# RuanJohn/Mava

Measured on AMD Instinct MI355X. Metric: env-steps/sec (whole node), ff_mappo RWARE tiny-4ag, higher is better.
Workload: dtype f32 via 2 x f16 split operands on the MFMA (3 products, f32 accumulate); 1 GPU; ff_mappo RWARE tiny-4ag-shaped synthetic obs, 4096 envs/GPU (update_batch_size=1 x num_envs=4096), rollout_length=128, ppo_epochs=4, num_minibatches=2, agents=4, obs=70/264, actions=5, one step = one PPO update = 524288 env-steps per GPU; parallelism=dp1

## Files before the change

mava_amd/csrc/ppo_train_h2.hip:

```cpp
#include "h2_core.h"
#include "ppo_train_task.h"
#include "ctx.h"

#include <type_traits>

#ifndef MAVA_GW_DEPTH
#define MAVA_GW_DEPTH 0
#endif
#define GW_DEPTH MAVA_GW_DEPTH
#ifndef MAVA_GW_DEPTH_WIDE
#define MAVA_GW_DEPTH_WIDE 0
#endif

namespace {

using namespace h2;

constexpr int STATS_BLOCKS = 128;

#ifdef MAVA_STAMPS
#define STAMP_DECL unsigned long long st_prev = __builtin_readcyclecounter(), st_acc[16] = {0, 0, 0, 0, 0, 0, 0, 0, 0, 0, 0, 0, 0, 0, 0, 0};
#define STAMP(i)                                                    \
  do {                                                              \
    __builtin_amdgcn_sched_barrier(0);                              \
    const unsigned long long st_now = __builtin_readcyclecounter(); \
    st_acc[i] += st_now - st_prev;                                  \
    st_prev = st_now;                                               \
    __builtin_amdgcn_sched_barrier(0);                              \
  } while (0)
#else
#define STAMP_DECL
#define STAMP(i)
#endif

struct H2Layout {
  int h1, dz2, dz1, w2, xs, xs_plane, xs_row, dy, yp, agg, small, end;
};

template <int NO, int S1, bool WIDE>
H2Layout make_h2_layout(bool actor) {
  constexpr int KT1 = (S1 + 1) / 2;
  H2Layout L;
  L.h1 = 0;
  L.dz2 = L.h1 + IMG_BYTES;
  L.dz1 = L.dz2 + IMG_BYTES;
  L.w2 = L.dz1 + IMG_BYTES;
  L.xs = L.w2 + 4 * IMG_BYTES;
  L.xs_row = 2 * 32 * KT1 + 16;
  L.xs_plane = 32 * L.xs_row;
  L.dy = L.xs + (WIDE ? 1 : 2) * 2 * L.xs_plane;
  L.yp = actor ? L.dz2 : L.dz1;
  L.agg = L.dy + (actor ? 2 * DY_PLANE : 0);
  L.small = L.agg + 8 * 33 * 4;
  L.small = (L.small + 15) & ~15;
  L.end = L.small + (128 + 32 + 16 + 128) * 4;
  return L;
}
constexpr int W2_PLANE = 128 * SW_ROW;
constexpr int W1_RING = 3;

template <int STEPS>
__global__ __launch_bounds__(256) void pack_w1_kernel(const float* __restrict__ P, int din, uint4* __restrict__ out, float scale) {
  pack_w1_body<STEPS>(P, din, out, threadIdx.x, scale);
}

template <int NO, int S1, bool ACTOR, bool WIDE, int XV, int ROLE>
__device__ __forceinline__ void h2_body(const TrainTask& tk, const H2Layout& L, const uint4* __restrict__ w1p, u8* lds) {
  static_assert(!WIDE || S1 % W1_RING == 0, "WIDE: S1 must be a multiple of the W1 ring depth");
  static_assert((ROLE == 0) == !WIDE, "roles 1 / 2 belong to WIDE launches");
  constexpr bool CHAIN = ROLE != 2, LOADER = ROLE != 1;
#if defined(MAVA_NO_W2_RESIDENT) || defined(MAVA_W2_RESIDENT_P4)
  constexpr bool W2_RESIDENT = false;
#else
  constexpr bool W2_RESIDENT = !WIDE && NO <= 16;
#endif
#ifdef MAVA_W2_RESIDENT_P4
  constexpr bool W2_RES4 = !WIDE && ACTOR && NO <= 16;
#else
  constexpr bool W2_RES4 = false;
#endif
  constexpr int NTHR = WIDE ? 512 : 256;
  constexpr float WS = ACTOR ? 1.0f : W_SCALE_CRITIC, WU = 1.0f / WS;
  constexpr int KT1 = (S1 + 1) / 2;
  u8* const H1I = lds + L.h1;
  u8* const DZ2I = lds + L.dz2;
  u8* const DZ1I = lds + L.dz1;
  u8* const H2I = lds + L.dz1;
  u8* const W2I = lds + L.w2;
  u8* const DYI = lds + L.dy;
  float* const YP = reinterpret_cast<float*>(lds + L.yp);
  float* const AGG = reinterpret_cast<float*>(lds + L.agg);
  float* const B2s = reinterpret_cast<float*>(lds + L.small);
  float* const B3s = B2s + 128;
  float* const misc = B3s + 32;
  float* const W3s = misc + 16;
  const int xs_row = L.xs_row, xs_plane = L.xs_plane;

  int tid = threadIdx.x & 255;
  int lane = tid & 63, w = tid >> 6, h = lane >> 5, r = lane & 31;
  int srow = tid >> 3, l8 = tid & 7;
  const int din = tk.din, no = tk.no;
  const long R = (!ACTOR && tk.agg > 1) ? (long)tk.Rb : (long)tk.Rb * tk.A;
  const float invR = 1.0f / (float)((long)tk.Rb * tk.A);
  constexpr int NPC = (32 * KT1 / XV + 7) / 8;
  constexpr int NR = NPC * XV;

  for (int i = threadIdx.x * 16; i < L.end; i += NTHR * 16) *reinterpret_cast<uint4*>(lds + i) = make_uint4(0, 0, 0, 0);
  __syncthreads();
  const float* const P = tk.params;
  const int oW2 = mlp_off_w2(din), oW3 = mlp_off_w3(din);
  if (CHAIN) {
    if (tid < 128) B2s[tid] = P[mlp_off_b2(din) + tid];
    if (tid < no) B3s[tid] = P[mlp_off_b3(din, no) + tid];
    if (!ACTOR && tid < 128) W3s[tid] = P[oW3 + tid];
    if (tid < (WIDE ? 32 : 64)) {
      const int b = tid >> 5, row = tid & 31;
      *reinterpret_cast<_Float16*>(lds + L.xs + b * 2 * xs_plane + row * xs_row + 2 * din) = (_Float16)1.0f;
    }
    {
      const int n = tid & 127, k0 = 64 * (tid >> 7);
      float carry = 0.0f;
#pragma unroll 8
      for (int k = k0; k < k0 + 64; ++k) {
        _Float16 x0, x1;
        split1_carry(P[oW2 + k * MLP_H + n] * WS, carry, x0, x1);
        const int o = sw_off(k, n >> 3) + 2 * (n & 7);
        *reinterpret_cast<_Float16*>(W2I + o) = x0;
        *reinterpret_cast<_Float16*>(W2I + W2_PLANE + o) = x1;
      }
    }
    if (ACTOR && tid == 0) {
      double s1 = 0.0, s2 = 0.0;
      for (int i = 0; i < STATS_BLOCKS; ++i) { s1 += tk.stats[2 * i]; s2 += tk.stats[2 * i + 1]; }
      const double mean = s1 / (double)R;
      double var = s2 / (double)R - mean * mean;
      if (var < 0.0) var = 0.0;
      misc[0] = (float)mean;
      misc[1] = 1.0f / ((float)sqrt(var) + 1e-8f);
    }
  }
  constexpr int S_LO = (WIDE && !CHAIN) ? S1 / 2 : 0, S_HI = (WIDE && CHAIN) ? S1 / 2 : S1, RL = S_HI - S_LO;
  static_assert(!WIDE || ((S1 / 2) % W1_RING == 0 && (S1 - S1 / 2) % W1_RING == 0), "WIDE: both halves must be multiples of the ring");
  constexpr int NW1 = WIDE ? W1_RING : (CHAIN ? S1 : 1);
  Frag W1f[NW1];
  const uint4* w1p_lane = w1p + 2 * (w * 64 + lane);
  typedef unsigned u32x4 __attribute__((ext_vector_type(4)));
  typedef const __attribute__((address_space(1))) u32x4* w1_gptr;
  auto w1_fetch = [&](int s) -> Frag {
    const w1_gptr g = (w1_gptr)w1p_lane;
    Frag f;
    f.hi = __builtin_bit_cast(half8, g[512 * s]);
    f.lo = __builtin_bit_cast(half8, g[512 * s + 1]);
    return f;
  };
  float w1_carry = 0.0f;
#pragma unroll
  for (int s = 0; s < (CHAIN ? NW1 : 0); ++s) {
    if (WIDE) {
      W1f[s] = w1_fetch(S_LO + s);
    } else {
      float v[8];
#pragma unroll
      for (int e = 0; e < 8; ++e) {
        const int k = 16 * s + 8 * h + e;
        v[e] = (k <= din) ? P[k * MLP_H + 32 * w + r] * WS : 0.0f;
      }
      W1f[s] = split8_carry(v, w1_carry);
    }
  }
  Frag W3h[2];
#pragma unroll
  for (int s = 0; s < ((CHAIN && ACTOR) ? 2 : 0); ++s) {
    float v[8];
#pragma unroll
    for (int e = 0; e < 8; ++e) {
      const int f = 32 * w + 16 * s + 8 * (e >> 2) + 4 * h + (e & 3);
      v[e] = (r < no) ? P[oW3 + f * no + r] * W3_SCALE : 0.0f;
    }
    W3h[s] = split8(v);
  }
  constexpr int ND = NO > 16 ? 2 : 1;
  Frag W3d[ND];
  if (CHAIN && ACTOR) {
#pragma unroll
    for (int s = 0; s < ND; ++s) {
      float v[8];
#pragma unroll
      for (int e = 0; e < 8; ++e) {
        const int o = 16 * s + 8 * h + e;
        v[e] = (o < no) ? P[oW3 + (32 * w + r) * no + o] * W3_SCALE : 0.0f;
      }
      W3d[s] = split8(v);
    }
  }
  __syncthreads();
  const float adv_mean = ACTOR ? misc[0] : 0.0f;
  const float adv_rstd = ACTOR ? misc[1] : 0.0f;

  f32x16 gW1[LOADER ? KT1 : 1], gW2[4], gW3;
#pragma unroll
  for (int t = 0; t < (LOADER ? KT1 : 1); ++t)
#pragma unroll
    for (int q = 0; q < 16; ++q) gW1[t][q] = 0.0f;
#pragma unroll
  for (int t = 0; t < 4; ++t)
#pragma unroll
    for (int q = 0; q < 16; ++q) gW2[t][q] = 0.0f;
#pragma unroll
  for (int q = 0; q < 16; ++q) gW3[q] = 0.0f;
  float ab2[16], aW3r[ACTOR ? 1 : 16];
#pragma unroll
  for (int q = 0; q < 16; ++q) ab2[q] = 0.0f;
#pragma unroll
  for (int q = 0; q < (ACTOR ? 1 : 16); ++q) aW3r[q] = 0.0f;
  float ab3 = 0.0f, loss_a = 0.0f, loss_b = 0.0f;

  constexpr int NP = ACTOR ? NO / 8 : 1;
  constexpr int GR = ACTOR ? 64 / NO : 32;
  const int lo = ACTOR ? (lane & (NO - 1)) : 0;
  auto loss_row = [&](int q) -> int { return ACTOR ? (8 * w + q * GR + lane / NO) : r; };
  const int slot = 2 * w + h;
  uint32_t slot_c = (!ACTOR && tk.agg > 1) ? (uint32_t)(slot < tk.agg ? slot : 0) : 0u;
  auto load_row = [&](long fr, int& act, float& f0, float& f1, uint32_t& m) {
    if (ACTOR) {
      act = tk.action[fr];
      f0 = tk.old_logp[fr];
      f1 = tk.adv[fr];
      const uint8_t* mk = (tk.mask != nullptr && lo < no) ? (tk.mask + fr * no + lo) : nullptr;
      m = 1u;
      if (mk != nullptr) m = *mk;
    } else {
      act = 0;
      const long fa = (tk.agg > 1) ? (long)((uint32_t)fr * (uint32_t)tk.agg + slot_c) : fr;
      f0 = tk.old_value[fa];
      f1 = tk.targets[fa];
      m = 0u;
    }
  };
  const uint32_t Au = (!ACTOR && tk.agg > 1) ? 1u : (uint32_t)tk.A;
  const uint32_t q_step = 32u * gridDim.x, b_step = q_step / Au, a_step = q_step % Au;
  const uint32_t b_last = (uint32_t)(R - 1) / Au, a_last = (uint32_t)(R - 1) % Au;
  struct Cursor { uint32_t q, b, a; };
  auto cursor_at = [&](int rr) {
    Cursor c;
    c.q = 32u * blockIdx.x + (uint32_t)rr;
    c.b = c.q / Au;
    c.a = c.q - c.b * Au;
    return c;
  };
  auto cursor_advance = [&](Cursor& c) {
    c.q += q_step; c.b += b_step; c.a += a_step;
    if (c.a >= Au) { c.a -= Au; c.b += 1u; }
  };
  auto cursor_gather = [&](const Cursor& c, int32_t& p_raw, uint32_t& a_out) {
    const bool in = c.q < (uint32_t)R;
    const uint32_t b = in ? c.b : b_last;
    a_out = in ? c.a : a_last;
    p_raw = tk.idx ? tk.idx[b] : (int32_t)(tk.idx_base + (long)b);
  };
  auto stage_row = [&](int32_t p_raw, uint32_t a) -> uint32_t {
    const uint32_t fr = (uint32_t)p_raw * Au + a;
    return (tk.xshare == 1) ? fr : ((uint32_t)tk.xshare == Au ? (uint32_t)p_raw : fr / (uint32_t)tk.xshare);
  };
  const int nv = din / XV;
  auto stage_issue = [&](uint32_t xrow_idx, float (&xr)[NR]) {
    const float* xrow = tk.x + (long)xrow_idx * din;
#pragma unroll
    for (int i = 0; i < NPC; ++i) {
      const int c = l8 + 8 * i;
      const int cc = (c < nv) ? c : 0;
      if (XV == 4) {
        const float4 v = reinterpret_cast<const float4*>(xrow)[cc];
        xr[4 * i] = v.x; xr[4 * i + 1] = v.y; xr[4 * i + 2] = v.z; xr[4 * i + 3] = v.w;
      } else if (XV == 2) {
        const float2 v = reinterpret_cast<const float2*>(xrow)[cc];
        xr[2 * i] = v.x; xr[2 * i + 1] = v.y;
      } else {
        xr[i] = xrow[cc];
      }
    }
  };
  u8* const xs_dummy = reinterpret_cast<u8*>(misc + 8);
  unsigned* const xflag = reinterpret_cast<unsigned*>(misc + 2);
  int tpar = 0;
  auto stage_commit = [&](auto hi_only_tag, auto flag_tag, u8* dst, const float (&xr)[NR], int flag_slot) {
    constexpr bool HI_ONLY = decltype(hi_only_tag)::value, FLAG = decltype(flag_tag)::value;
    u8* base = dst + srow * xs_row;
    uint32_t lo_any = 0;
#pragma unroll
    for (int i = 0; i < NPC; ++i) {
      const int c = l8 + 8 * i;
      const bool ok = c < nv;
      u8* qa = ok ? (base + 2 * XV * c) : xs_dummy;
      u8* qb = ok ? (base + xs_plane + 2 * XV * c) : xs_dummy;
      if (XV == 4) {
        half4 a, b;
#pragma unroll
        for (int e = 0; e < 4; ++e) { _Float16 x0, x1; split1(xr[4 * i + e], x0, x1); a[e] = x0; b[e] = x1; }
        *reinterpret_cast<half4*>(qa) = a;
        if constexpr (!HI_ONLY) *reinterpret_cast<half4*>(qb) = b;
        if constexpr (FLAG) {
          const uint2 bb = __builtin_bit_cast(uint2, b);
          lo_any |= (bb.x | bb.y) & 0x7FFF7FFFu;
        }
      } else if (XV == 2) {
        typedef _Float16 half2v __attribute__((ext_vector_type(2)));
        half2v a, b;
#pragma unroll
        for (int e = 0; e < 2; ++e) { _Float16 x0, x1; split1(xr[2 * i + e], x0, x1); a[e] = x0; b[e] = x1; }
        *reinterpret_cast<half2v*>(qa) = a;
        if constexpr (!HI_ONLY) *reinterpret_cast<half2v*>(qb) = b;
        if constexpr (FLAG) lo_any |= __builtin_bit_cast(uint32_t, b) & 0x7FFF7FFFu;
      } else {
        _Float16 x0, x1;
        split1(xr[i], x0, x1);
        *reinterpret_cast<_Float16*>(qa) = x0;
        if constexpr (!HI_ONLY) *reinterpret_cast<_Float16*>(qb) = x1;
        if constexpr (FLAG) lo_any |= (uint32_t)__builtin_bit_cast(uint16_t, x1) & 0x7FFFu;
      }
    }
    if constexpr (FLAG) {
      if (lo_any != 0) xflag[flag_slot] = 1u;
    }
  };
  using std::false_type;
  using std::true_type;
  constexpr bool VERSIONED = WIDE && !ACTOR;
  using versioned_tag = std::bool_constant<VERSIONED>;

  const long ntiles = (R + 31) / 32;
  long it = blockIdx.x;
  float xr[NR];
  int r_act[NP] = {}, n_act[NP] = {};
  float r_f0[NP] = {}, r_f1[NP] = {}, n_f0[NP] = {}, n_f1[NP] = {};
  uint32_t r_m[NP] = {}, n_m[NP] = {};
  Cursor cs = cursor_at(srow), cl[NP];
#pragma unroll
  for (int q = 0; q < NP; ++q) cl[q] = cursor_at(loss_row(q));
  int32_t ps_next = 0, pl_next[NP] = {};
  uint32_t as_next = 0, al_next[NP] = {};
  if (it < ntiles) {
    if (LOADER) {
      cursor_gather(cs, ps_next, as_next);
      stage_issue(stage_row(ps_next, as_next), xr);
    }
    if (CHAIN) {
#pragma unroll
      for (int q = 0; q < NP; ++q) {
        cursor_gather(cl[q], pl_next[q], al_next[q]);
        load_row((long)((uint32_t)pl_next[q] * Au + al_next[q]), r_act[q], r_f0[q], r_f1[q], r_m[q]);
      }
    }
    if (LOADER) {
      stage_commit(false_type{}, versioned_tag{}, lds + L.xs, xr, 0);
      cursor_advance(cs);
    }
    if (CHAIN) {
#pragma unroll
      for (int q = 0; q < NP; ++q) cursor_advance(cl[q]);
    }
    if (it + gridDim.x < ntiles) {
      if (LOADER) {
        cursor_gather(cs, ps_next, as_next);
        cursor_advance(cs);
      }
      if (CHAIN) {
#pragma unroll
        for (int q = 0; q < NP; ++q) cursor_gather(cl[q], pl_next[q], al_next[q]);
#pragma unroll
        for (int q = 0; q < NP; ++q) cursor_advance(cl[q]);
      }
    }
  }
  __syncthreads();

  SwRow rowB = sw_row(r, h);
  SwTr trS = sw_tr(lane);
  const int i16 = lane & 15, tq = i16 >> 2, tp = i16 & 3, g1 = (lane >> 4) & 1;
  int trX = (8 * h + tq) * xs_row + 2 * (16 * g1 + 4 * tp);
  const int trD = (8 * h + tq) * DY_ROW + 2 * (16 * g1 + 4 * tp);
  SwRow w2row = sw_row(32 * w + r, h);
  int buf = 0;
  Frag w2r[(W2_RESIDENT || W2_RES4) ? 8 : 1];
  if constexpr (W2_RESIDENT) {
#pragma unroll
    for (int s = 0; s < 8; ++s) w2r[s] = sw_read_tr(W2I, W2_PLANE, trS, s, w);
  }
  if constexpr (W2_RES4) {
#pragma unroll
    for (int s = 0; s < 8; ++s) w2r[s] = sw_read_row(W2I, W2_PLANE, w2row, s);
  }

  STAMP_DECL
  bool exact = false;
  unsigned n_exact = 0;
  auto tile_body = [&](auto exact_tag) __attribute__((always_inline)) {
    constexpr bool EXACT = decltype(exact_tag)::value;
    static_assert(!EXACT || VERSIONED, "the exact-input loop belongs to the wide critic");
    STAMP(14);
    const bool valid = (it * 32 + r) < R;
    const long itn = it + gridDim.x;
    const bool have_next = itn < ntiles;
    if constexpr (EXACT && LOADER) {
      if (tid == 0) xflag[tpar ^ 1] = 0u;
    }
    uint32_t xrow_next = LOADER ? stage_row(ps_next, as_next) : 0u;
    uint32_t fr_next[NP];
#pragma unroll
    for (int q = 0; q < NP; ++q) fr_next[q] = CHAIN ? ((uint32_t)pl_next[q] * Au + al_next[q]) : 0u;
    if (LOADER) asm volatile("" : "+v"(xrow_next));
    if (CHAIN) {
#pragma unroll
      for (int q = 0; q < NP; ++q) asm volatile("" : "+v"(fr_next[q]));
    }
    const u8* const XSI = lds + L.xs + (EXACT ? tpar : 2 * buf) * xs_plane;

    f32x16 acc;
    uint32_t relu1 = 0;
    if constexpr (WIDE) asm volatile("" : "+v"(w1p_lane));
    if constexpr (CHAIN || WIDE) {
#pragma unroll
    for (int q = 0; q < 16; ++q) acc[q] = 0.0f;
    if constexpr (WIDE && !CHAIN) {
#pragma unroll
      for (int s = 0; s < NW1; ++s) W1f[s] = w1_fetch(S_LO + s);
    }
    Frag xb;
    xb.hi = *reinterpret_cast<const half8*>(XSI + r * xs_row + 16 * h + 32 * S_LO);
    if constexpr (!EXACT) xb.lo = *reinterpret_cast<const half8*>(XSI + xs_plane + r * xs_row + 16 * h + 32 * S_LO);
#pragma unroll
    for (int j = 0; j < RL; ++j) {
      const Frag b = xb;
      if (j + 1 < RL) {
        xb.hi = *reinterpret_cast<const half8*>(XSI + r * xs_row + 16 * h + 32 * (S_LO + j + 1));
        if constexpr (!EXACT) xb.lo = *reinterpret_cast<const half8*>(XSI + xs_plane + r * xs_row + 16 * h + 32 * (S_LO + j + 1));
      }
      if constexpr (EXACT) {
        acc = __builtin_amdgcn_mfma_f32_32x32x16_f16(W1f[j % NW1].lo, b.hi, acc, 0, 0, 0);
        acc = __builtin_amdgcn_mfma_f32_32x32x16_f16(W1f[j % NW1].hi, b.hi, acc, 0, 0, 0);
      } else {
        acc = mfma3(W1f[j % NW1], b, acc);
      }
      if (WIDE) {
        if (j >= 1 && j - 1 + W1_RING < RL) W1f[(j - 1) % NW1] = w1_fetch(S_LO + j - 1 + W1_RING);
      }
      __builtin_amdgcn_sched_barrier(0);
    }
    }
    if constexpr (WIDE) {
      float4* const xch = reinterpret_cast<float4*>(DZ2I) + (w * 4) * 64 + lane;
      if constexpr (LOADER) {
#pragma unroll
        for (int g = 0; g < 4; ++g) xch[g * 64] = make_float4(acc[4 * g], acc[4 * g + 1], acc[4 * g + 2], acc[4 * g + 3]);
      }
      __syncthreads();
      if constexpr (CHAIN) {
#pragma unroll
        for (int g = 0; g < 4; ++g) {
          const float4 v = xch[g * 64];
          acc[4 * g] += v.x; acc[4 * g + 1] += v.y; acc[4 * g + 2] += v.z; acc[4 * g + 3] += v.w;
        }
      }
    }
    if constexpr (CHAIN) {
    STAMP(0);
#pragma unroll
    for (int q = 0; q < 16; ++q) {
      acc[q] = fmaxf(ACTOR ? acc[q] : acc[q] * WU, 0.0f);
      relu1 |= (acc[q] > 0.0f) ? (1u << q) : 0u;
    }
    {
      half4 ph[4], pl[4];
      sw_write_image(H1I, r, w, h, acc, ph, pl);
    }
    }
    STAMP(1);
    if constexpr (WIDE && LOADER) {
      stage_issue(have_next ? xrow_next : 0u, xr);
    }
    if constexpr (WIDE && CHAIN) {
#pragma unroll
      for (int q = 0; q < NP; ++q) {
        asm volatile("" : "+v"(fr_next[q]));
        asm volatile("" : "+v"(cl[q].q), "+v"(cl[q].b), "+v"(cl[q].a));
      }
      asm volatile("" : "+v"(slot_c));
    }
    if constexpr (WIDE && CHAIN) {
      if (have_next) {
        const bool more = itn + gridDim.x < ntiles;
        Cursor c_old[NP];
        if (more) {
#pragma unroll
          for (int q = 0; q < NP; ++q) { c_old[q] = cl[q]; cursor_advance(cl[q]); }
        }
        __builtin_amdgcn_sched_barrier(0);
#pragma unroll
        for (int q = 0; q < NP; ++q) load_row((long)fr_next[q], n_act[q], n_f0[q], n_f1[q], n_m[q]);
        __builtin_amdgcn_sched_barrier(0);
        if (more) {
#pragma unroll
          for (int q = 0; q < NP; ++q) cursor_gather(c_old[q], pl_next[q], al_next[q]);
        }
      }
    } else if (have_next) {
      if (LOADER && !WIDE) stage_issue(xrow_next, xr);
      const bool more = itn + gridDim.x < ntiles;
      if (more) {
        if (LOADER) {
          cursor_gather(cs, ps_next, as_next);
          cursor_advance(cs);
        }
        if (CHAIN) {
          Cursor c_old[NP];
#pragma unroll
          for (int q = 0; q < NP; ++q) { c_old[q] = cl[q]; cursor_advance(cl[q]); }
          __builtin_amdgcn_sched_barrier(0);
#pragma unroll
          for (int q = 0; q < NP; ++q) cursor_gather(c_old[q], pl_next[q], al_next[q]);
        }
      }
      if (CHAIN) {
#pragma unroll
        for (int q = 0; q < NP; ++q) load_row((long)fr_next[q], n_act[q], n_f0[q], n_f1[q], n_m[q]);
      }
    }
    if constexpr (WIDE && CHAIN) {
      __builtin_amdgcn_sched_barrier(0);
#pragma unroll
      for (int s2 = 0; s2 < NW1; ++s2) W1f[s2] = w1_fetch(S_LO + s2);
      __builtin_amdgcn_sched_barrier(0);
    }
    STAMP(2);
    __syncthreads();
    STAMP(3);

    f32x16 h2;
    uint32_t relu2 = 0;
    if constexpr (CHAIN) {
#pragma unroll
    for (int q = 0; q < 16; ++q) h2[q] = B2s[32 * w + (q & 3) + 8 * (q >> 2) + 4 * h] * WS;
    {
      Frag an;
      if constexpr (!W2_RESIDENT) an = sw_read_tr(W2I, W2_PLANE, trS, 0, w);
      Frag bn = sw_read_row(H1I, SW_PLANE, rowB, 0);
#pragma unroll
      for (int s = 0; s < 8; ++s) {
        const Frag a = W2_RESIDENT ? w2r[s] : an, b = bn;
        if (s + 1 < 8) {
          if constexpr (!W2_RESIDENT) an = sw_read_tr(W2I, W2_PLANE, trS, s + 1, w);
          bn = sw_read_row(H1I, SW_PLANE, rowB, s + 1);
        }
        h2 = mfma3(a, b, h2);
        __builtin_amdgcn_sched_barrier(0);
      }
    }
    STAMP(4);
#pragma unroll
    for (int q = 0; q < 16; ++q) {
      h2[q] = fmaxf(ACTOR ? h2[q] : h2[q] * WU, 0.0f);
      relu2 |= (h2[q] > 0.0f) ? (1u << q) : 0u;
    }
    if (!ACTOR) {
      float4 w3g[4];
#pragma unroll
      for (int g = 0; g < 4; ++g) w3g[g] = *reinterpret_cast<const float4*>(W3s + 32 * w + 4 * h + 8 * g);
      float part = 0.0f;
#pragma unroll
      for (int q = 0; q < 16; ++q) {
        const float4 t = w3g[q >> 2];
        const float w3 = (q & 3) == 0 ? t.x : (q & 3) == 1 ? t.y : (q & 3) == 2 ? t.z : t.w;
        part = fmaf(h2[q], w3, part);
      }
      part += __shfl_xor(part, 32, 64);
      if (h == 0) YP[(w * 32 + r) * (NO + 1)] = part;
    } else {
      half4 ph[4], pl[4];
      sw_write_image(H2I, r, w, h, h2, ph, pl);
      f32x16 yacc;
#pragma unroll
      for (int q = 0; q < 16; ++q) yacc[q] = 0.0f;
#pragma unroll
      for (int s = 0; s < 2; ++s) {
        Frag b;
        b.hi = __builtin_shufflevector(ph[2 * s], ph[2 * s + 1], 0, 1, 2, 3, 4, 5, 6, 7);
        b.lo = __builtin_shufflevector(pl[2 * s], pl[2 * s + 1], 0, 1, 2, 3, 4, 5, 6, 7);
        yacc = mfma3(W3h[s], b, yacc);
      }
#pragma unroll
      for (int q = 0; q < 16; ++q) {
        const int o = (q & 3) + 8 * (q >> 2) + 4 * h;
        if ((q & 3) + 8 * (q >> 2) < NO) {
          if (o < NO) YP[(w * 32 + r) * (NO + 1) + o] = yacc[q] * W3_UNSCALE;
        }
      }
    }
    }
    STAMP(5);
    __syncthreads();
    STAMP(6);
    if constexpr (EXACT && LOADER) {
      stage_commit(true_type{}, true_type{}, lds + L.xs + (tpar ^ 1) * xs_plane, xr, tpar ^ 1);
    }

    f32x16 dz;
    float dy0 = 0.0f;
    if constexpr (CHAIN) {
    if (ACTOR) {
      const float lo_c = 1.0f - tk.clip_eps, hi_c = 1.0f + tk.clip_eps;
#pragma unroll
      for (int q = 0; q < NP; ++q) {
        const int row = loss_row(q);
        const bool rvalid = (it * 32 + row) < R;
        const float* yp = YP + row * (NO + 1) + lo;
        const float y = (((yp[0] + yp[32 * (NO + 1)]) + yp[2 * 32 * (NO + 1)]) + yp[3 * 32 * (NO + 1)]) + B3s[lo];
        const bool legal = (lo < no) && (r_m[q] != 0u);
        const float z = legal ? y : -FLT_MAX;
        auto fmax_op = [](float a, float b) { return fmaxf(a, b); };
        auto add_op = [](float a, float b) { return a + b; };
        const float mx = group_allreduce<NO>(z, fmax_op);
        const float se = group_allreduce<NO>(expf(z - mx), add_op);
        const float logp = (mx == -FLT_MAX) ? ((lo < no) ? -logf((float)no) : -FLT_MAX) : z - (mx + logf(se));
        const float pr = expf(logp);
        const float ent = group_allreduce<NO>((pr > 0.0f) ? -(pr * logp) : 0.0f, add_op);
        const int act = r_act[q];
        const float lp = group_allreduce<NO>((lo == act) ? logp : 0.0f, add_op);
        const float gae = (r_f1[q] - adv_mean) * adv_rstd;
        const float ratio = expf(lp - r_f0[q]);
        const float rc = fminf(fmaxf(ratio, lo_c), hi_c);
        const float l1 = ratio * gae, l2 = rc * gae;
        const float pg = -fminf(l1, l2);
        const bool inside = (ratio >= lo_c) && (ratio <= hi_c);
        const float g1 = (l1 < l2) ? 1.0f : ((l1 == l2) ? 0.5f : 0.0f);
        const float g2 = inside ? (1.0f - g1) : 0.0f;
        const float dlp = rvalid ? (-(g1 + g2) * gae * ratio) : 0.0f;
        const float ec = rvalid ? tk.ent_coef : 0.0f;
        const float oh = (lo == act) ? 1.0f : 0.0f;
        const float pl2 = (pr > 0.0f) ? logp : 0.0f;
        float dyo = dlp * (oh - pr) + ec * pr * (pl2 + ent);
        if (z == -FLT_MAX) dyo = 0.0f;
        _Float16 da, db;
        split1(dyo, da, db);
        *reinterpret_cast<_Float16*>(DYI + row * DY_ROW + 2 * lo) = da;
        *reinterpret_cast<_Float16*>(DYI + DY_PLANE + row * DY_ROW + 2 * lo) = db;
        ab3 += dyo;
        if (rvalid && lo == 0) {
          loss_a += pg * invR;
          loss_b += ent * invR;
        }
      }
    } else {
      const float* yp = YP + r * (NO + 1);
      const float v = (((yp[0] + yp[32 * (NO + 1)]) + yp[2 * 32 * (NO + 1)]) + yp[3 * 32 * (NO + 1)]) + B3s[0];
      const float ov = r_f0[0], tg = r_f1[0];
      const float diff = v - ov;
      const float vclip = ov + fminf(fmaxf(diff, -tk.clip_eps), tk.clip_eps);
      const float e1 = v - tg, e2 = vclip - tg;
      const float l1 = e1 * e1, l2 = e2 * e2;
      const bool inside = (diff >= -tk.clip_eps) && (diff <= tk.clip_eps);
      const float g1 = (l1 > l2) ? 1.0f : ((l1 == l2) ? 0.5f : 0.0f);
      const float g2 = inside ? (1.0f - g1) : 0.0f;
      dy0 = valid ? (tk.vf_coef * (g1 * e1 + g2 * e2)) : 0.0f;
      if (tk.agg > 1) {
        const bool mine = valid && slot < tk.agg;
        dy0 = mine ? dy0 : 0.0f;
        if (mine) {
          loss_a += 0.5f * fmaxf(l1, l2) * invR;
          ab3 += dy0;
        }
        AGG[slot * 33 + r] = dy0;
      } else if (valid && w == 0 && h == 0) {
        loss_a += 0.5f * fmaxf(l1, l2) * invR;
        ab3 += dy0;
      }
    }
    }
    STAMP(7);
    __syncthreads();
    STAMP(15);
    if constexpr (CHAIN) {
    if (ACTOR) {
#pragma unroll
      for (int s = 0; s < 2; ++s) {
        const Frag a = read_tr_frag(DYI + trD + 16 * s * DY_ROW, DY_PLANE, DY_ROW);
        const Frag b = sw_read_tr(H2I, SW_PLANE, trS, s, w);
        gW3 = mfma3(a, b, gW3);
      }
#pragma unroll
      for (int q = 0; q < 16; ++q) dz[q] = 0.0f;
#pragma unroll
      for (int s = 0; s < ND; ++s) {
        const Frag b = read_row_frag(DYI, DY_PLANE, r * DY_ROW + 32 * s + 16 * h);
        dz = mfma3(W3d[s], b, dz);
      }
#pragma unroll
      for (int q = 0; q < 16; ++q) {
        dz[q] = ((relu2 >> q) & 1u) ? dz[q] * W3_UNSCALE : 0.0f;
        ab2[q] += dz[q];
      }
    } else {
      float4 w3g[4];
#pragma unroll
      for (int g = 0; g < 4; ++g) w3g[g] = *reinterpret_cast<const float4*>(W3s + 32 * w + 4 * h + 8 * g);
      if (tk.agg > 1) {
        float av[8];
#pragma unroll
        for (int a = 0; a < 8; ++a) av[a] = AGG[a * 33 + r];
        float sum = 0.0f;
#pragma unroll
        for (int a = 0; a < 8; ++a) sum += av[a];
        dy0 = sum;
      }
#pragma unroll
      for (int q = 0; q < 16; ++q) {
        const float4 t = w3g[q >> 2];
        const float w3 = (q & 3) == 0 ? t.x : (q & 3) == 1 ? t.y : (q & 3) == 2 ? t.z : t.w;
        const float v = w3 * dy0;
        dz[q] = ((relu2 >> q) & 1u) ? v : 0.0f;
        ab2[q] += dz[q];
        aW3r[q] = fmaf(h2[q], dy0, aW3r[q]);
      }
    }
    {
      half4 ph[4], pl[4];
      sw_write_image(DZ2I, r, w, h, dz, ph, pl);
    }
    }
    STAMP(8);
    __syncthreads();
    STAMP(9);

    auto do_gw2 = [&]() {
      constexpr int D2 = WIDE ? 0 : GW_DEPTH;
      if constexpr (D2 > 0) {
        const Frag b0 = sw_read_tr(DZ2I, SW_PLANE, trS, 0, w), b1 = sw_read_tr(DZ2I, SW_PLANE, trS, 1, w);
        Frag a[D2 > 0 ? D2 : 1];
#pragma unroll
        for (int i = 0; i < D2; ++i) a[i] = sw_read_tr(H1I, SW_PLANE, trS, i >> 2, i & 3);
#pragma unroll
        for (int i = 0; i < 8; ++i) {
          const Frag cur = a[i % (D2 > 0 ? D2 : 1)];
          if (i + D2 < 8) a[i % (D2 > 0 ? D2 : 1)] = sw_read_tr(H1I, SW_PLANE, trS, (i + D2) >> 2, (i + D2) & 3);
          gW2[i & 3] = mfma3(cur, (i >> 2) ? b1 : b0, gW2[i & 3]);
          __builtin_amdgcn_sched_barrier(0);
        }
      } else {
#pragma unroll
        for (int s = 0; s < 2; ++s) {
          const Frag b = sw_read_tr(DZ2I, SW_PLANE, trS, s, w);
#pragma unroll
          for (int t = 0; t < 4; ++t) {
            const Frag a = sw_read_tr(H1I, SW_PLANE, trS, s, t);
            gW2[t] = mfma3(a, b, gW2[t]);
            if (t & 1) __builtin_amdgcn_sched_barrier(0);
          }
        }
      }
    };
    if constexpr (CHAIN) {
#pragma unroll
      for (int q = 0; q < 16; ++q) acc[q] = 0.0f;
      Frag an;
      if constexpr (!W2_RES4) an = sw_read_row(W2I, W2_PLANE, w2row, 0);
      Frag bn = sw_read_row(DZ2I, SW_PLANE, rowB, 0);
#pragma unroll
      for (int s = 0; s < 8; ++s) {
        const Frag a = W2_RES4 ? w2r[s] : an, b = bn;
        if (s + 1 < 8) {
          if constexpr (!W2_RES4) an = sw_read_row(W2I, W2_PLANE, w2row, s + 1);
          bn = sw_read_row(DZ2I, SW_PLANE, rowB, s + 1);
        }
        acc = mfma3(a, b, acc);
        __builtin_amdgcn_sched_barrier(0);
      }
#pragma unroll
      for (int q = 0; q < 16; ++q) acc[q] = ((relu1 >> q) & 1u) ? (ACTOR ? acc[q] : acc[q] * WU) : 0.0f;
      half4 ph[4], pl[4];
      sw_write_image(DZ1I, r, w, h, acc, ph, pl);
    }
    if constexpr (!WIDE) {
      if (have_next) stage_commit(false_type{}, false_type{}, lds + L.xs + (buf ^ 1) * 2 * xs_plane, xr, 0);
    }
    STAMP(10);
    if constexpr (!WIDE) do_gw2();
    STAMP(11);
    __syncthreads();
    STAMP(12);
    if constexpr (WIDE && CHAIN) do_gw2();
    if constexpr (LOADER) {
      constexpr int NPR = 2 * KT1;
      constexpr int D1 = WIDE ? MAVA_GW_DEPTH_WIDE : GW_DEPTH;
      if constexpr (EXACT) {
#pragma unroll
        for (int s = 0; s < 2; ++s) {
          const Frag b = sw_read_tr(DZ1I, SW_PLANE, trS, s, w);
#pragma unroll
          for (int t = 0; t < KT1; ++t) {
            const half8 a = read_tr8(XSI + trX + 16 * s * xs_row + 2 * (32 * t), xs_row);
            const f32x16 c = __builtin_amdgcn_mfma_f32_32x32x16_f16(a, b.lo, gW1[t], 0, 0, 0);
            gW1[t] = __builtin_amdgcn_mfma_f32_32x32x16_f16(a, b.hi, c, 0, 0, 0);
            if (t & 1) __builtin_amdgcn_sched_barrier(0);
          }
        }
      } else if constexpr (D1 > 0) {
        constexpr int DP = D1 < NPR ? D1 : NPR;
        const Frag b0 = sw_read_tr(DZ1I, SW_PLANE, trS, 0, w), b1 = sw_read_tr(DZ1I, SW_PLANE, trS, 1, w);
        Frag a[DP > 0 ? DP : 1];
#pragma unroll
        for (int i = 0; i < DP; ++i) a[i] = read_tr_frag(XSI + trX + 16 * (i / KT1) * xs_row + 2 * (32 * (i % KT1)), xs_plane, xs_row);
#pragma unroll
        for (int i = 0; i < NPR; ++i) {
          const Frag cur = a[i % (DP > 0 ? DP : 1)];
          if (i + DP < NPR)
            a[i % (DP > 0 ? DP : 1)] = read_tr_frag(XSI + trX + 16 * ((i + DP) / KT1) * xs_row + 2 * (32 * ((i + DP) % KT1)), xs_plane, xs_row);
          gW1[i % KT1] = mfma3(cur, (i / KT1) ? b1 : b0, gW1[i % KT1]);
          __builtin_amdgcn_sched_barrier(0);
        }
      } else {
#pragma unroll
        for (int s = 0; s < 2; ++s) {
          const Frag b = sw_read_tr(DZ1I, SW_PLANE, trS, s, w);
#pragma unroll
          for (int t = 0; t < KT1; ++t) {
            const Frag a = read_tr_frag(XSI + trX + 16 * s * xs_row + 2 * (32 * t), xs_plane, xs_row);
            gW1[t] = mfma3(a, b, gW1[t]);
            if (t & 1) __builtin_amdgcn_sched_barrier(0);
          }
        }
      }
    }
    STAMP(13);
    if constexpr (WIDE) {
      __syncthreads();
      if constexpr (EXACT) {
        exact = __builtin_amdgcn_readfirstlane((int)xflag[tpar ^ 1]) == 0;
        ++n_exact;
      } else {
        if constexpr (LOADER) {
          stage_commit(false_type{}, false_type{}, lds + L.xs, xr, 0);
        }
        __syncthreads();
      }
    }
    if constexpr (CHAIN) {
#pragma unroll
      for (int q = 0; q < NP; ++q) { r_act[q] = n_act[q]; r_f0[q] = n_f0[q]; r_f1[q] = n_f1[q]; r_m[q] = n_m[q]; }
    }
  };
  if constexpr (VERSIONED) {
    exact = __builtin_amdgcn_readfirstlane((int)xflag[0]) == 0 && tk.force_xlo == 0;
    if (exact && it < ntiles) {
      if (CHAIN && tid < 32) *reinterpret_cast<_Float16*>(lds + L.xs + xs_plane + tid * xs_row + 2 * din) = (_Float16)1.0f;
    }
    for (; it < ntiles && exact; it += gridDim.x, tpar ^= 1) tile_body(true_type{});
    asm volatile("" : "+v"(tid), "+v"(lane), "+v"(w), "+v"(h), "+v"(r), "+v"(trS.b0), "+v"(trS.b1), "+v"(trS.q64));
    if constexpr (LOADER) asm volatile("" : "+v"(srow), "+v"(l8), "+v"(trX));
    if constexpr (CHAIN) asm volatile("" : "+v"(rowB.base), "+v"(rowB.hx), "+v"(w2row.base), "+v"(w2row.hx));
    if (n_exact != 0 && it < ntiles) {
      if constexpr (LOADER) stage_commit(false_type{}, false_type{}, lds + L.xs, xr, 0);
      if (CHAIN && tid < 32) *reinterpret_cast<_Float16*>(lds + L.xs + xs_plane + tid * xs_row + 2 * din) = (_Float16)0.0f;
      __syncthreads();
    }
  }
  for (; it < ntiles; it += gridDim.x, buf ^= (WIDE ? 0 : 1)) tile_body(false_type{});
#ifdef MAVA_STAMPS
  if (tk.stamps != nullptr && blockIdx.x == 0 && lane == 0) {
    for (int i = 0; i < 16; ++i) tk.stamps[((ROLE == 2 ? 4 : 0) + w) * 16 + i] = st_acc[i];
  }
#endif

  __syncthreads();
  if constexpr (VERSIONED && CHAIN) {
    if (tid == 0 && tk.exact_tiles != nullptr) atomicAdd(tk.exact_tiles, (unsigned long long)n_exact);
  }
  float* slab = tk.slab + (long)blockIdx.x * tk.slab_stride;
  const int oB2 = mlp_off_b2(din), oB3 = mlp_off_b3(din, no);
  const int Pn = mlp_param_count(din, no);
  if constexpr (LOADER) {
#pragma unroll
    for (int t = 0; t < KT1; ++t)
#pragma unroll
      for (int q = 0; q < 16; ++q) {
        const int k = mlp_feat(t, q, h);
        if (k <= din) slab[k * MLP_H + 32 * w + r] = gW1[t][q] * invR;
      }
  }
  if constexpr (CHAIN) {
#pragma unroll
    for (int t = 0; t < 4; ++t)
#pragma unroll
      for (int q = 0; q < 16; ++q) slab[oW2 + mlp_feat(t, q, h) * MLP_H + 32 * w + r] = gW2[t][q] * invR;
#pragma unroll
    for (int q = 0; q < 16; ++q) {
      float v = ab2[q];
#pragma unroll
      for (int m = 1; m < 32; m <<= 1) v += __shfl_xor(v, m, 64);
      if (r == 0) slab[oB2 + 32 * w + (q & 3) + 8 * (q >> 2) + 4 * h] = v * invR;
    }
  }
  float* red = reinterpret_cast<float*>(lds + L.h1);
  if constexpr (!CHAIN) {
    __syncthreads();
  } else if (ACTOR) {
#pragma unroll
    for (int q = 0; q < 16; ++q) {
      const int o = (q & 3) + 8 * (q >> 2) + 4 * h;
      if (o < no) slab[oW3 + (32 * w + r) * no + o] = gW3[q] * invR;
    }
    float v = ab3;
#pragma unroll
    for (int m = NO; m < 64; m <<= 1) v += __shfl_xor(v, m, 64);
    if (lane < NO) red[w * NO + lane] = v;
    for (int o = 32; o > 0; o >>= 1) {
      loss_a += __shfl_down(loss_a, o, 64);
      loss_b += __shfl_down(loss_b, o, 64);
    }
    if (lane == 0) { red[4 * NO + 2 * w] = loss_a; red[4 * NO + 2 * w + 1] = loss_b; }
    __syncthreads();
    if (tid < no) slab[oB3 + tid] = (((red[tid] + red[NO + tid]) + red[2 * NO + tid]) + red[3 * NO + tid]) * invR;
    if (tid == 0) {
      slab[Pn] = ((red[4 * NO] + red[4 * NO + 2]) + red[4 * NO + 4]) + red[4 * NO + 6];
      slab[Pn + 1] = ((red[4 * NO + 1] + red[4 * NO + 3]) + red[4 * NO + 5]) + red[4 * NO + 7];
    }
  } else {
#pragma unroll
    for (int q = 0; q < 16; ++q) {
      float v = aW3r[q];
#pragma unroll
      for (int m = 1; m < 32; m <<= 1) v += __shfl_xor(v, m, 64);
      if (r == 0) slab[oW3 + 32 * w + (q & 3) + 8 * (q >> 2) + 4 * h] = v * invR;
    }
    float v = ab3, l = loss_a;
    for (int o = 32; o > 0; o >>= 1) {
      v += __shfl_down(v, o, 64);
      l += __shfl_down(l, o, 64);
    }
    if (lane == 0) { red[2 * w] = v; red[2 * w + 1] = l; }
    __syncthreads();
    if (tid == 0) {
      slab[oB3] = (((red[0] + red[2]) + red[4]) + red[6]) * invR;
      slab[Pn] = ((red[1] + red[3]) + red[5]) + red[7];
      slab[Pn + 1] = 0.0f;
    }
  }
}

template <int NO, int S1, bool ACTOR, bool WIDE, int XV>
__global__ __launch_bounds__(WIDE ? 512 : 256, WIDE ? 2 : 1) void ppo_train_h2_kernel(TrainTask tk, H2Layout L,
                                                                                     const uint4* __restrict__ w1p) {
  extern __shared__ __attribute__((aligned(16))) u8 lds[];
  if constexpr (WIDE) {
    if (threadIdx.x < 256) {
      h2_body<NO, S1, ACTOR, WIDE, XV, 1>(tk, L, w1p, lds);
    } else {
      h2_body<NO, S1, ACTOR, WIDE, XV, 2>(tk, L, w1p, lds);
    }
  } else {
    h2_body<NO, S1, ACTOR, WIDE, XV, 0>(tk, L, w1p, lds);
  }
}

template <int NO, int S1, bool ACTOR, bool WIDE, int XV>
int launch_h2(mava_ctx* ctx, const TrainTask& tk, int n_slab, hipStream_t s) {
  const H2Layout L = make_h2_layout<NO, S1, WIDE>(ACTOR);
  MAVA_ARG_CHECK(L.end <= 163840, 8, "ppo_train_h2: %d bytes of LDS exceed the 160 KiB of a CU", L.end);
  static bool attr_set = false;
  if (!attr_set) {
    MAVA_HIP_CHECK(hipFuncSetAttribute((const void*)ppo_train_h2_kernel<NO, S1, ACTOR, WIDE, XV>,
                                       hipFuncAttributeMaxDynamicSharedMemorySize, L.end));
    attr_set = true;
  }
  const uint4* w1p = nullptr;
  if (WIDE) {
    void*& slot = ctx->w1_split[ACTOR ? 0 : 1];
    if (slot == nullptr) MAVA_HIP_CHECK(hipMalloc(&slot, W1_SPLIT_BYTES));
    uint4* const buf = static_cast<uint4*>(slot);
    const int kind = ACTOR ? 0 : 1;
    int& fresh = ctx->w1_fresh[kind];
    const bool keyed = ctx->w1_key_params[kind] == tk.params && ctx->w1_key_din[kind] == tk.din && ctx->w1_key_steps[kind] == S1;
    if (!(fresh && keyed)) {
      hipLaunchKernelGGL((pack_w1_kernel<S1>), dim3(1), dim3(256), 0, s, tk.params, tk.din, buf, ACTOR ? 1.0f : W_SCALE_CRITIC);
      MAVA_LAUNCH_CHECK();
    }
    fresh = 0;
    w1p = buf;
    if (ctx->exact_tiles == nullptr) {
      void* word = nullptr;
      MAVA_HIP_CHECK(hipMalloc(&word, sizeof(unsigned long long)));
      ctx->exact_tiles = static_cast<unsigned long long*>(word);
      MAVA_HIP_CHECK(hipMemsetAsync(word, 0, sizeof(unsigned long long), s));
    }
  }
  TrainTask tkl = tk;
  tkl.exact_tiles = WIDE ? ctx->exact_tiles : nullptr;
  g_train_last_instance = train_instance_id(2, ACTOR, false, WIDE, NO, S1, XV);
  hipLaunchKernelGGL((ppo_train_h2_kernel<NO, S1, ACTOR, WIDE, XV>), dim3(n_slab), dim3(WIDE ? 512 : 256), L.end, s, tkl, L,
                     w1p);
  MAVA_LAUNCH_CHECK();
  return MAVA_OK;
}

template <int NO, int S1, bool ACTOR, bool WIDE>
int dispatch_xv(mava_ctx* ctx, const TrainTask& tk, int n_slab, hipStream_t s) {
  const uintptr_t a = (uintptr_t)tk.x;
  if constexpr (WIDE) {
    if (tk.din % 4 == 0 && a % 16 == 0) return launch_h2<NO, S1, ACTOR, WIDE, 4>(ctx, tk, n_slab, s);
  } else {
    if (tk.din % 2 == 0 && a % 8 == 0) return launch_h2<NO, S1, ACTOR, WIDE, 2>(ctx, tk, n_slab, s);
  }
  return launch_h2<NO, S1, ACTOR, WIDE, 1>(ctx, tk, n_slab, s);
}

template <int NO, bool ACTOR>
int dispatch_s1(mava_ctx* ctx, const TrainTask& tk, int n_slab, hipStream_t s) {
  const int s1 = (tk.din + 1 + 15) / 16;
  switch (s1) {
#ifndef MAVA_FAST_BUILD
    case 1: return dispatch_xv<NO, 1, ACTOR, false>(ctx, tk, n_slab, s);
    case 2: return dispatch_xv<NO, 2, ACTOR, false>(ctx, tk, n_slab, s);
    case 3: return dispatch_xv<NO, 3, ACTOR, false>(ctx, tk, n_slab, s);
    case 4: return dispatch_xv<NO, 4, ACTOR, false>(ctx, tk, n_slab, s);
    case 6: return dispatch_xv<NO, 6, ACTOR, false>(ctx, tk, n_slab, s);
    case 7: case 8: case 9: case 10: case 11: case 12: return dispatch_xv<NO, 12, ACTOR, true>(ctx, tk, n_slab, s);
#endif
    case 5: return dispatch_xv<NO, 5, ACTOR, false>(ctx, tk, n_slab, s);
    case 13: case 14: case 15: case 16: case 17: case 18: return dispatch_xv<NO, 18, ACTOR, true>(ctx, tk, n_slab, s);
    default: return 1;
  }
}

}

static int h2_dispatch(mava_ctx* ctx, const TrainTask& tk, int n_slab, bool actor, hipStream_t s) {
  if (actor) {
    if (tk.action_f != nullptr) return 1;
    if (tk.no <= 8) return dispatch_s1<8, true>(ctx, tk, n_slab, s);
#ifndef MAVA_FAST_BUILD
    if (tk.no <= 16) return dispatch_s1<16, true>(ctx, tk, n_slab, s);
    return dispatch_s1<32, true>(ctx, tk, n_slab, s);
#else
    return 1;
#endif
  }
  return dispatch_s1<1, false>(ctx, tk, n_slab, s);
}

int mava_train_h2_launch(mava_ctx* ctx, const TrainTask& tk_in, int n_slab, bool actor, hipStream_t s) {
  TrainTask tk = tk_in;
  tk.force_xlo = (ctx->train_variant & 2) != 0;
  if ((ctx->train_variant & 1) == 0) {
    const int rc8 = mava_train_w8_launch(tk, n_slab, actor, s);
    if (rc8 <= 0) {
      if (rc8 == 0) { ++ctx->h2_launches; ++ctx->w8_launches; }
      return rc8;
    }
  }
  const int rc = h2_dispatch(ctx, tk, n_slab, actor, s);
  if (rc == 0) ++ctx->h2_launches;
  return rc;
}
```

Baseline: 79.77 million env-steps/s.

## Precompute next tile's layer-1 forward on loader waves during current tile backward

For the wide critic's exact-input loop, the loader role now runs the next tile's first-layer MFMA products early. The work is split into three chunks placed in the idle gaps between the current tile's backward phases, and W1 is streamed through a small register ring. By default all S1 steps move to the loader, which writes the ReLU'd h1 image and a relu mask to a new LDS slot, so the chain role skips its own layer-1 pass. This is meant to take the layer-1 forward off the critical path, at the cost of extra registers, more LDS and more complex staging around the exact/non-exact transition.

```diff
diff --git a/mava_amd/csrc/ppo_train_h2.hip b/mava_amd/csrc/ppo_train_h2.hip
--- a/mava_amd/csrc/ppo_train_h2.hip
+++ b/mava_amd/csrc/ppo_train_h2.hip
@@ -10,6 +10,12 @@
 #define GW_DEPTH MAVA_GW_DEPTH
 #ifndef MAVA_GW_DEPTH_WIDE
 #define MAVA_GW_DEPTH_WIDE 0
+#endif
+#ifndef MAVA_P1_EARLY_HALVES
+#define MAVA_P1_EARLY_HALVES 2
+#endif
+#ifndef MAVA_P1_EARLY_RING
+#define MAVA_P1_EARLY_RING 3
 #endif
 
 namespace {
@@ -34,7 +40,7 @@
 #endif
 
 struct H2Layout {
-  int h1, dz2, dz1, w2, xs, xs_plane, xs_row, dy, yp, agg, small, end;
+  int h1, dz2, dz1, w2, xs, xs_plane, xs_row, dy, yp, agg, small, relu, end;
 };
 
 template <int NO, int S1, bool WIDE>
@@ -53,7 +59,8 @@
   L.agg = L.dy + (actor ? 2 * DY_PLANE : 0);
   L.small = L.agg + 8 * 33 * 4;
   L.small = (L.small + 15) & ~15;
-  L.end = L.small + (128 + 32 + 16 + 128) * 4;
+  L.relu = L.small + (128 + 32 + 16 + 128) * 4;
+  L.end = L.relu + (WIDE ? 256 * 4 : 0);
   return L;
 }
 constexpr int W2_PLANE = 128 * SW_ROW;
@@ -94,6 +101,11 @@
   float* const B3s = B2s + 128;
   float* const misc = B3s + 32;
   float* const W3s = misc + 16;
+  uint32_t* const RELU1 = reinterpret_cast<uint32_t*>(lds + L.relu);
+  constexpr bool VERSIONED = WIDE && !ACTOR;
+  constexpr int P1_EARLY = VERSIONED ? MAVA_P1_EARLY_HALVES * (S1 / 2) : 0;
+  static_assert(MAVA_P1_EARLY_HALVES >= 0 && MAVA_P1_EARLY_HALVES <= 2, "P1_EARLY is 0, S1 / 2 or S1");
+  constexpr bool EARLY = P1_EARLY > 0, EARLY_ALL = EARLY && P1_EARLY == S1;
   const int xs_row = L.xs_row, xs_plane = L.xs_plane;
 
   int tid = threadIdx.x & 255;
@@ -155,7 +167,7 @@
   };
   float w1_carry = 0.0f;
 #pragma unroll
-  for (int s = 0; s < (CHAIN ? NW1 : 0); ++s) {
+  for (int s = 0; s < ((CHAIN && !EARLY_ALL) ? NW1 : 0); ++s) {
     if (WIDE) {
       W1f[s] = w1_fetch(S_LO + s);
     } else {
@@ -325,7 +337,6 @@
   };
   using std::false_type;
   using std::true_type;
-  constexpr bool VERSIONED = WIDE && !ACTOR;
   using versioned_tag = std::bool_constant<VERSIONED>;
 
   const long ntiles = (R + 31) / 32;
@@ -394,9 +405,45 @@
   STAMP_DECL
   bool exact = false;
   unsigned n_exact = 0;
+  constexpr int ER = MAVA_P1_EARLY_RING, SB = S1 - P1_EARLY;
+  constexpr int GB = P1_EARLY / 9, GC = GB + (P1_EARLY * 7) / 18;
+  f32x16 eC, eL;
+  Frag W1e[(EARLY && LOADER) ? ER : 1];
+  auto early_fill = [&]() __attribute__((always_inline)) {
+#pragma unroll
+    for (int g = 0; g < ER && g < P1_EARLY; ++g) W1e[g] = w1_fetch(SB + g);
+  };
+  auto early_steps = [&](auto g0_tag, auto g1_tag, const u8* xsi) __attribute__((always_inline)) {
+    constexpr int G0 = decltype(g0_tag)::value, G1 = decltype(g1_tag)::value;
+    if constexpr (G0 < G1) {
+      half8 xh = *reinterpret_cast<const half8*>(xsi + r * xs_row + 16 * h + 32 * (SB + G0));
+#pragma unroll
+      for (int g = G0; g < G1; ++g) {
+        const half8 b = xh;
+        if (g + 1 < G1) xh = *reinterpret_cast<const half8*>(xsi + r * xs_row + 16 * h + 32 * (SB + g + 1));
+        if (g == 0 || SB + g == S1 / 2) {
+#pragma unroll
+          for (int q = 0; q < 16; ++q) {
+            if (SB + g < S1 / 2) eC[q] = 0.0f; else eL[q] = 0.0f;
+          }
+        }
+        if (SB + g < S1 / 2) {
+          eC = __builtin_amdgcn_mfma_f32_32x32x16_f16(W1e[g % ER].lo, b, eC, 0, 0, 0);
+          eC = __builtin_amdgcn_mfma_f32_32x32x16_f16(W1e[g % ER].hi, b, eC, 0, 0, 0);
+        } else {
+          eL = __builtin_amdgcn_mfma_f32_32x32x16_f16(W1e[g % ER].lo, b, eL, 0, 0, 0);
+          eL = __builtin_amdgcn_mfma_f32_32x32x16_f16(W1e[g % ER].hi, b, eL, 0, 0, 0);
+        }
+        if (g >= 1 && g - 1 + ER < P1_EARLY) W1e[(g - 1) % ER] = w1_fetch(SB + g - 1 + ER);
+        __builtin_amdgcn_sched_barrier(0);
+      }
+    }
+  };
+  uint32_t xrow_keep = 0;
   auto tile_body = [&](auto exact_tag) __attribute__((always_inline)) {
     constexpr bool EXACT = decltype(exact_tag)::value;
     static_assert(!EXACT || VERSIONED, "the exact-input loop belongs to the wide critic");
+    constexpr bool XE = EXACT && EARLY;
     STAMP(14);
     const bool valid = (it * 32 + r) < R;
     const long itn = it + gridDim.x;
@@ -414,11 +461,12 @@
       for (int q = 0; q < NP; ++q) asm volatile("" : "+v"(fr_next[q]));
     }
     const u8* const XSI = lds + L.xs + (EXACT ? tpar : 2 * buf) * xs_plane;
+    if constexpr (XE && LOADER) xrow_keep = xrow_next;
 
     f32x16 acc;
     uint32_t relu1 = 0;
     if constexpr (WIDE) asm volatile("" : "+v"(w1p_lane));
-    if constexpr (CHAIN || WIDE) {
+    if constexpr ((CHAIN || WIDE) && !(XE && (LOADER || EARLY_ALL))) {
 #pragma unroll
     for (int q = 0; q < 16; ++q) acc[q] = 0.0f;
     if constexpr (WIDE && !CHAIN) {
@@ -447,9 +495,26 @@
       __builtin_amdgcn_sched_barrier(0);
     }
     }
-    if constexpr (WIDE) {
+    if constexpr (XE && EARLY_ALL && LOADER) {
+#pragma unroll
+      for (int q = 0; q < 16; ++q) {
+        acc[q] = fmaxf((eC[q] + eL[q]) * WU, 0.0f);
+        relu1 |= (acc[q] > 0.0f) ? (1u << q) : 0u;
+      }
+      __builtin_amdgcn_sched_barrier(0);
+      stage_issue(have_next ? xrow_next : 0u, xr);
+      __builtin_amdgcn_sched_barrier(0);
+      half4 ph[4], pl[4];
+      sw_write_image(H1I, r, w, h, acc, ph, pl);
+      RELU1[tid] = relu1;
+    }
+    if constexpr (WIDE && !(XE && EARLY_ALL)) {
       float4* const xch = reinterpret_cast<float4*>(DZ2I) + (w * 4) * 64 + lane;
       if constexpr (LOADER) {
+        if constexpr (XE) {
+          acc = eL;
+          stage_issue(have_next ? xrow_next : 0u, xr);
+        }
 #pragma unroll
         for (int g = 0; g < 4; ++g) xch[g * 64] = make_float4(acc[4 * g], acc[4 * g + 1], acc[4 * g + 2], acc[4 * g + 3]);
       }
@@ -462,7 +527,7 @@
         }
       }
     }
-    if constexpr (CHAIN) {
+    if constexpr (CHAIN && !(XE && EARLY_ALL)) {
     STAMP(0);
 #pragma unroll
     for (int q = 0; q < 16; ++q) {
@@ -475,7 +540,7 @@
     }
     }
     STAMP(1);
-    if constexpr (WIDE && LOADER) {
+    if constexpr (WIDE && LOADER && !XE) {
       stage_issue(have_next ? xrow_next : 0u, xr);
     }
     if constexpr (WIDE && CHAIN) {
@@ -525,7 +590,7 @@
         for (int q = 0; q < NP; ++q) load_row((long)fr_next[q], n_act[q], n_f0[q], n_f1[q], n_m[q]);
       }
     }
-    if constexpr (WIDE && CHAIN) {
+    if constexpr (WIDE && CHAIN && !(XE && EARLY_ALL)) {
       __builtin_amdgcn_sched_barrier(0);
 #pragma unroll
       for (int s2 = 0; s2 < NW1; ++s2) W1f[s2] = w1_fetch(S_LO + s2);
@@ -534,6 +599,11 @@
     STAMP(2);
     __syncthreads();
     STAMP(3);
+    if constexpr (XE && LOADER) {
+      stage_commit(true_type{}, true_type{}, lds + L.xs + (tpar ^ 1) * xs_plane, xr, tpar ^ 1);
+      early_fill();
+    }
+    if constexpr (XE && EARLY_ALL && CHAIN) relu1 = RELU1[tid];
 
     f32x16 h2;
     uint32_t relu2 = 0;
@@ -599,7 +669,8 @@
     STAMP(5);
     __syncthreads();
     STAMP(6);
-    if constexpr (EXACT && LOADER) {
+    if constexpr (XE && LOADER) early_steps(std::integral_constant<int, 0>{}, std::integral_constant<int, GB>{}, lds + L.xs + (tpar ^ 1) * xs_plane);
+    if constexpr (EXACT && LOADER && !XE) {
       stage_commit(true_type{}, true_type{}, lds + L.xs + (tpar ^ 1) * xs_plane, xr, tpar ^ 1);
     }
 
@@ -678,6 +749,7 @@
     STAMP(7);
     __syncthreads();
     STAMP(15);
+    if constexpr (XE && LOADER) early_steps(std::integral_constant<int, GB>{}, std::integral_constant<int, GC>{}, lds + L.xs + (tpar ^ 1) * xs_plane);
     if constexpr (CHAIN) {
     if (ACTOR) {
 #pragma unroll
@@ -781,6 +853,7 @@
     if constexpr (!WIDE) {
       if (have_next) stage_commit(false_type{}, false_type{}, lds + L.xs + (buf ^ 1) * 2 * xs_plane, xr, 0);
     }
+    if constexpr (XE && LOADER) early_steps(std::integral_constant<int, GC>{}, std::integral_constant<int, P1_EARLY>{}, lds + L.xs + (tpar ^ 1) * xs_plane);
     STAMP(10);
     if constexpr (!WIDE) do_gw2();
     STAMP(11);
@@ -852,14 +925,28 @@
     if (exact && it < ntiles) {
       if (CHAIN && tid < 32) *reinterpret_cast<_Float16*>(lds + L.xs + xs_plane + tid * xs_row + 2 * din) = (_Float16)1.0f;
     }
+    if constexpr (EARLY && LOADER) {
+      early_fill();
+      early_steps(std::integral_constant<int, 0>{}, std::integral_constant<int, P1_EARLY>{}, lds + L.xs);
+    }
     for (; it < ntiles && exact; it += gridDim.x, tpar ^= 1) tile_body(true_type{});
     asm volatile("" : "+v"(tid), "+v"(lane), "+v"(w), "+v"(h), "+v"(r), "+v"(trS.b0), "+v"(trS.b1), "+v"(trS.q64));
     if constexpr (LOADER) asm volatile("" : "+v"(srow), "+v"(l8), "+v"(trX));
     if constexpr (CHAIN) asm volatile("" : "+v"(rowB.base), "+v"(rowB.hx), "+v"(w2row.base), "+v"(w2row.hx));
     if (n_exact != 0 && it < ntiles) {
-      if constexpr (LOADER) stage_commit(false_type{}, false_type{}, lds + L.xs, xr, 0);
+      if constexpr (LOADER) {
+        if constexpr (EARLY) {
+          asm volatile("" : "+v"(xrow_keep));
+          stage_issue(xrow_keep, xr);
+        }
+        stage_commit(false_type{}, false_type{}, lds + L.xs, xr, 0);
+      }
       if (CHAIN && tid < 32) *reinterpret_cast<_Float16*>(lds + L.xs + xs_plane + tid * xs_row + 2 * din) = (_Float16)0.0f;
       __syncthreads();
+    }
+    if constexpr (EARLY_ALL && CHAIN) {
+#pragma unroll
+      for (int s = 0; s < NW1; ++s) W1f[s] = w1_fetch(S_LO + s);
     }
   }
   for (; it < ntiles; it += gridDim.x, buf ^= (WIDE ? 0 : 1)) tile_body(false_type{});
```

Result: faster. 81.67 million env-steps/s, median of 6 (+2.4%).
